# lifunudt/CORB-SLAM

Measured on AMD Instinct MI355X. Metric: stereo frames/sec ORB extract+match, higher is better.
Workload: dtype u8; 1 GPU; configs[1]: ORB extract+match, synthetic 1241x376 stereo stream, 2000 feat/frame, 8 levels x1.2, FAST 20/7; warmup_frames_per_gpu=2560, batches_in_flight=1, distinct_frames=64, parallelism=1 client per GPU, replicas (no collective), inputs=resident in HBM

## Files before the change

corb-slam_amd/csrc/corb_internal.h:

```cpp
#pragma once
#include <hip/hip_runtime.h>
#include <stdint.h>
#include <stddef.h>
#include "../../include/corb_accel.h"

#include <stdlib.h>
#ifdef CORB_DEV
static inline const char* corb_dev_env(const char* name) { return getenv(name); }
#else
static inline const char* corb_dev_env(const char*) { return nullptr; }
#endif

#define CORB_MAX_LEVELS 16
#define CORB_EDGE_THRESHOLD 19
#define CORB_MIN_BORDER 16
#define CORB_HALF_PATCH 15
#define CORB_PATCH_SIZE 31
#define CORB_TH_HIGH 100
#define CORB_TH_LOW 50
#define CORB_HISTO_LENGTH 30

struct CorbLevel {
    int w, h, pitch;
    int plane_off;
    int nCols, nRows, wCell, hCell;
    int maxBX, maxBY;
    int cell_base;
    int cell_cap;
    int cand_base;
    int cand_cap;
    int quota;
    int kp_base, kp_cap;
    int nIni;
    int node_cap;
    int blur_tile_base, blur_tiles_x, blur_tiles_y;
    int resize_tab_off;
    int resize_rec_off;
    float scale;
    float hX;
    int patch_size;
};

struct CorbFastCell {
    uint32_t src_off;
    uint32_t org;
    uint32_t dim;
    uint32_t lane;
};

#define CORB_BLUR_T 64
#define CORB_MAX_PARTS 4

struct CorbOrbParams {
    int nlevels, n_images;
    int img_base;
    int ini_th, min_th;
    int cells_per_image, cand_per_image, kp_per_image, out_cap;
    int blur_tiles_per_image;
    int node_cap_max, ncell_max;
    int fast_tp, fast_th;
    int pyr_strips;
    short pyr_r0[8][CORB_MAX_LEVELS], pyr_r1[8][CORB_MAX_LEVELS];
    int pyr_ctiles;
    short pyr_g0[8][CORB_MAX_LEVELS], pyr_g1[8][CORB_MAX_LEVELS];
    size_t arena_per_image;
    uint8_t* pyr;
    uint8_t* blur;
    int* cell_count;
    uint32_t* cand;
    uint32_t* keys;
    uint16_t* key_node;
    uint32_t* kp;
    int* kp_count;
    const short* resize_tab;
    const int2* resize_rec;
    const CorbFastCell* fast_cells;
    CorbKeyPoint* out_kp;
    uint8_t* out_desc;
    int* out_count;
    int* status;
    CorbLevel lv[CORB_MAX_LEVELS];
};

struct CorbStereoParams {
    int n_frames, nlevels;
    int frame_base;
    float bf, mb;
    float scale[CORB_MAX_LEVELS], inv_scale[CORB_MAX_LEVELS];
    int rows0;
    float* u_right;
    float* depth;
    int* sad;
    int* n_matched;
    int* row_off;
    int2* row_idx;
    int row_cap;
    int2* left_range;
};

#ifdef __HIPCC__
__device__ __forceinline__ void corb_xcd_remap(int& unit, int& img)
{
    const unsigned nx = gridDim.x, nimg = gridDim.y;
    const unsigned B = blockIdx.x + nx * blockIdx.y;
    const unsigned g = B / (8u * nx), r = B - g * 8u * nx;
    const unsigned in_group = min(8u, nimg - 8u * g);
    img = (int)(8u * g + r % in_group);
    unit = (int)(r / in_group);
}
#endif

struct CorbStereoDeviceFrame { const CorbKeyPoint* kp; const uint8_t* desc; const float* u_right; const float* depth; const int* count; int cap; hipStream_t stream; int device; };
struct CorbStereo;
int corb_stereo_device_frame(CorbStereo* h, int frame, CorbStereoDeviceFrame* out);
struct CorbRgbd;
int corb_rgbd_device_frame(CorbRgbd* h, int frame, CorbStereoDeviceFrame* out);

struct CorbProfiler;
void corb_orb_device_init();
void corb_launch_ingest(const uint8_t* stage, int w, int h, int n_images, uint8_t* plane, int pitch, size_t image_stride, hipStream_t stream);
void corb_launch_stereo_pack(const CorbOrbParams& p, const CorbStereoParams& s, int frame_base, int n_frames, uint8_t* out, const CorbStereoFrameLayout& lay, hipStream_t stream, struct CorbProfiler* prof);
void corb_launch_orb_pipeline(const CorbOrbParams& p, int img_base, int n_images, size_t octree_lds, hipStream_t stream, CorbProfiler* prof, hipEvent_t after_fast = nullptr);
void corb_launch_candidates(const CorbOrbParams* dp, int img, int level, CorbKeyPoint* out, int cap, int* n_out, hipStream_t stream);
void corb_launch_stereo(const CorbOrbParams& p, const CorbStereoParams& s, int frame_base, int n_frames, hipStream_t stream, CorbProfiler* prof);
size_t corb_octree_lds_bytes(int node_cap_max, int ncell_max);

#ifdef __HIPCC__
#include <hip/hip_ext.h>
#define CORB_LAUNCH(prof, name, kernel, grid, block, lds, stream, ...) do { \
// ... 19 lines not shown
```

corb-slam_amd/csrc/corb_orb.cpp:

```cpp
#include "corb_internal.h"
#include "orb_handle.h"
#include <cmath>
#include <cfloat>
#include <cstdio>
#include <cstdarg>
#include <cstring>
#include <mutex>
#include <map>
#include <vector>

static thread_local char g_err[512] = "";
void corb_set_error(const char* fmt, ...)
{
    va_list ap; va_start(ap, fmt); vsnprintf(g_err, sizeof(g_err), fmt, ap); va_end(ap);
}
extern "C" const char* corb_last_error(void) { return g_err; }
extern "C" int corb_version(void) { return 100; }
extern "C" int corb_abi_version(void) { return CORB_ABI_VERSION; }
extern "C" int corb_device_count(void)
{
    int n = 0;
    if (hipGetDeviceCount(&n) != hipSuccess) return 0;
    return n;
}
// ... 11 lines not shown

static inline int cv_round(double v) { return (int)lrint(v); }
static inline int cv_floor(double v) { int i = cv_round(v); float d = (float)(v - i); return i - (d < 0); }
static inline int cv_ceil(double v) { int i = cv_round(v); float d = (float)(i - v); return i + (d < 0); }
static inline short sat_short(int v) { return (short)(v < -32768 ? -32768 : v > 32767 ? 32767 : v); }

int corb_select_device(int device)
{
    int n = 0;
    if (hipGetDeviceCount(&n) != hipSuccess || n <= 0) { corb_set_error("no HIP device visible"); return CORB_ERR_NO_DEVICE; }
    if (device < 0 || device >= n) { corb_set_error("device %d out of range (%d visible)", device, n); return CORB_ERR_ARG; }
    HIPCHK(hipSetDevice(device));
    static std::mutex mu; static bool inited[64] = {false};
    std::lock_guard<std::mutex> lk(mu);
    if (device < 64 && !inited[device]) {
        hipDeviceProp_t prop;
        HIPCHK(hipGetDeviceProperties(&prop, device));
        if (strncmp(prop.gcnArchName, "gfx950", 6) != 0) {
            corb_set_error("device %d is %s; libcorb_accel is built for gfx950 only", device, prop.gcnArchName);
            return CORB_ERR_NO_DEVICE;
        }
        corb_orb_device_init();
        HIPCHK(hipGetLastError());
        inited[device] = true;
    }
    return CORB_OK;
}

static void build_resize_tables(int sw, int sh, int dw, int dh, short* tab)
{
    short* xofs = tab, * xa0 = tab + dw, * xa1 = tab + 2 * dw;
    short* ys0 = tab + 3 * dw, * ys1 = ys0 + dh, * yb0 = ys1 + dh, * yb1 = yb0 + dh;
    const double inv_scale_x = (double)dw / sw, inv_scale_y = (double)dh / sh;
    const double scale_x = 1. / inv_scale_x, scale_y = 1. / inv_scale_y;
    for (int dx = 0; dx < dw; dx++) {
        float fx = (float)((dx + 0.5) * scale_x - 0.5);
        int sx = cv_floor(fx);
        fx -= sx;
        if (sx < 0) { fx = 0; sx = 0; }
        if (sx + 1 >= sw) { if (sx >= sw - 1) { fx = 0; sx = sw - 1; } }
        xofs[dx] = (short)sx;
        xa0[dx] = sat_short(cv_round((1.f - fx) * 2048));
        xa1[dx] = sat_short(cv_round(fx * 2048));
        if (sx + 1 >= sw) { xa0[dx] = 2048; xa1[dx] = 0; }
    }
    for (int dy = 0; dy < dh; dy++) {
        float fy = (float)((dy + 0.5) * scale_y - 0.5);
        int sy = cv_floor(fy);
        fy -= sy;
        yb0[dy] = sat_short(cv_round((1.f - fy) * 2048));
        yb1[dy] = sat_short(cv_round(fy * 2048));
        ys0[dy] = (short)(sy < 0 ? 0 : (sy < sh ? sy : sh - 1));
        ys1[dy] = (short)(sy + 1 < 0 ? 0 : (sy + 1 < sh ? sy + 1 : sh - 1));
    }
}

extern "C" int corb_orb_create(const CorbOrbConfig* cfg, CorbOrb** out)
{
    if (!cfg || !out) { corb_set_error("null argument"); return CORB_ERR_ARG; }
    *out = nullptr;
    if (cfg->nlevels < 1 || cfg->nlevels > CORB_MAX_LEVELS || cfg->nfeatures < 1 || cfg->max_images < 1 ||
        cfg->width < 1 || cfg->height < 1 || cfg->width > 4000 || cfg->height > 4000 || !(cfg->scale_factor > 1.0f) ||
        cfg->min_th_fast < 1 || cfg->ini_th_fast < cfg->min_th_fast || cfg->ini_th_fast > 255) {
        corb_set_error("invalid CorbOrbConfig"); return CORB_ERR_ARG;
    }
    int rc = corb_select_device(cfg->device);
    if (rc != CORB_OK) return rc;
    CorbOrb* h = new CorbOrb();
    h->cfg = *cfg;
    const int nl = cfg->nlevels;
    h->scale[0] = 1.0f; h->sigma2[0] = 1.0f;
    for (int i = 1; i < nl; i++) { h->scale[i] = h->scale[i - 1] * cfg->scale_factor; h->sigma2[i] = h->scale[i] * h->scale[i]; }
    for (int i = 0; i < nl; i++) { h->inv_scale[i] = 1.0f / h->scale[i]; h->inv_sigma2[i] = 1.0f / h->sigma2[i]; }
    {
        float factor = 1.0f / cfg->scale_factor;
        float nDesired = cfg->nfeatures * (1 - factor) / (1 - (float)pow((double)factor, (double)nl));
        int sum = 0;
        for (int level = 0; level < nl - 1; level++) { h->quota[level] = cv_round(nDesired); sum += h->quota[level]; nDesired *= factor; }
        h->quota[nl - 1] = std::max(cfg->nfeatures - sum, 0);
        int v, v0, vmax = cv_floor(CORB_HALF_PATCH * sqrtf(2.f) / 2 + 1), vmin = cv_ceil(CORB_HALF_PATCH * sqrtf(2.f) / 2);
        const double hp2 = CORB_HALF_PATCH * CORB_HALF_PATCH;
        for (v = 0; v <= vmax; ++v) h->umax[v] = cv_round(sqrt(hp2 - v * v));
        for (v = CORB_HALF_PATCH, v0 = 0; v >= vmin; --v) { while (h->umax[v0] == h->umax[v0 + 1]) ++v0; h->umax[v] = v0; ++v0; }
        static const int expect[16] = {15, 15, 15, 15, 14, 14, 14, 13, 13, 12, 11, 10, 9, 8, 6, 3};
        for (int i = 0; i < 16; i++) if (h->umax[i] != expect[i]) { corb_set_error("umax table mismatch"); delete h; return CORB_ERR_ARG; }
    }
    CorbOrbParams& p = h->p;
    memset(&p, 0, sizeof(p));
    p.nlevels = nl; p.n_images = cfg->max_images; p.ini_th = cfg->ini_th_fast; p.min_th = cfg->min_th_fast;
    size_t arena = 0; int cells = 0, cands = 0, kps = 0, tiles = 0, tab_off = 0, rec_off = 0;
    for (int l = 0; l < nl; l++) {
        CorbLevel& L = p.lv[l];
        L.w = cv_round((float)cfg->width * h->inv_scale[l]);
        L.h = cv_round((float)cfg->height * h->inv_scale[l]);
        L.pitch = (L.w + 63) & ~63;
        L.plane_off = (int)arena;
        arena += ((size_t)L.pitch * L.h + 255) & ~(size_t)255;
        L.maxBX = L.w - CORB_EDGE_THRESHOLD + 3; L.maxBY = L.h - CORB_EDGE_THRESHOLD + 3;
        const float width = (float)(L.maxBX - CORB_MIN_BORDER), height = (float)(L.maxBY - CORB_MIN_BORDER);
        L.nCols = (int)(width / 30.f); L.nRows = (int)(height / 30.f);
        if (L.nCols < 1 || L.nRows < 1) { corb_set_error("level %d (%dx%d) too small for the 30-px FAST grid", l, L.w, L.h); delete h; return CORB_ERR_ARG; }
        L.wCell = (int)ceilf(width / L.nCols); L.hCell = (int)ceilf(height / L.nRows);
        if (L.wCell > 64 || L.hCell > 64) { corb_set_error("FAST cell %dx%d exceeds the LDS tile", L.wCell, L.hCell); delete h; return CORB_ERR_ARG; }
        L.cell_base = cells; cells += L.nCols * L.nRows;
        L.cell_cap = ((L.wCell + 1) / 2) * ((L.hCell + 1) / 2);
        L.cand_base = cands; L.cand_cap = L.nCols * L.nRows * L.cell_cap; cands += L.cand_cap;
// ... 20 lines not shown
    h->octree_lds = corb_octree_lds_bytes(p.node_cap_max, p.ncell_max);
    if (h->octree_lds > 160 * 1024) { corb_set_error("quadtree needs %zu B of LDS (> 160 KiB): nfeatures too large", h->octree_lds); delete h; return CORB_ERR_ARG; }
    if (p.node_cap_max > 65535) { corb_set_error("nfeatures too large"); delete h; return CORB_ERR_ARG; }
    const size_t NI = (size_t)cfg->max_images;
    short* d_tab = nullptr;
#define DA(ptr, n) do { rc = dalloc(h, &(ptr), (n)); if (rc != CORB_OK) { corb_orb_destroy(h); return rc; } } while (0)
    DA(p.pyr, NI * arena); DA(p.blur, NI * arena);
    DA(p.cell_count, NI * cells); DA(p.cand, NI * cands); DA(p.keys, NI * cands); DA(p.key_node, NI * cands);
    DA(p.kp, NI * kps); DA(p.kp_count, NI * CORB_MAX_LEVELS);
    DA(p.out_kp, NI * p.out_cap); DA(p.out_desc, NI * p.out_cap * 32); DA(p.out_count, NI); DA(p.status, NI);
    DA(d_tab, (size_t)tab_off);
    int2* d_rec = nullptr;
    DA(d_rec, (size_t)rec_off + 4);
    CorbFastCell* d_cells = nullptr;
    DA(d_cells, (size_t)cells);
    DA(h->dp, 1);
#undef DA
    p.resize_tab = d_tab;
    p.resize_rec = d_rec;
    p.fast_cells = d_cells;
    {
        std::vector<CorbFastCell> fc((size_t)cells);
        for (int l = 0; l < nl; l++) {
            const CorbLevel& L = p.lv[l];
            for (int c = 0; c < L.nCols * L.nRows; c++) {
                const int ci = c / L.nCols, cj = c - ci * L.nCols;
                const int iniX = CORB_MIN_BORDER + cj * L.wCell, iniY = CORB_MIN_BORDER + ci * L.hCell;
                const int cw = std::min(iniX + L.wCell + 6, L.maxBX) - iniX, ch = std::min(iniY + L.hCell + 6, L.maxBY) - iniY;
                CorbFastCell& f = fc[(size_t)L.cell_base + c];
                f.org = (uint32_t)(iniX + 3 - CORB_MIN_BORDER) | ((uint32_t)(iniY + 3 - CORB_MIN_BORDER) << 12) | ((uint32_t)l << 24);
                if (cw < 7 || ch < 7) { f.src_off = 0; f.org |= 0x80000000u; f.dim = 0; f.lane = 0; continue; }
                const int gx0 = iniX - 1, a = gx0 & 3, ng = (cw - 6 + 3) >> 2;
                f.src_off = (uint32_t)L.plane_off + (uint32_t)iniY * (uint32_t)L.pitch + (uint32_t)(gx0 - a);
                f.dim = (uint32_t)cw | ((uint32_t)ch << 8) | ((uint32_t)(64 / ng) << 16) | ((uint32_t)ng << 24);
                f.lane = (uint32_t)((65536 + ng - 1) / ng) | ((uint32_t)((a + cw) >> 2) << 20);
            }
        }
        if (hipMemcpy(d_cells, fc.data(), fc.size() * sizeof(CorbFastCell), hipMemcpyHostToDevice) != hipSuccess) { corb_set_error("FAST cell table upload failed"); corb_orb_destroy(h); return CORB_ERR_HIP; }
    }
    {
        std::vector<short> tab(tab_off);
        for (int l = 1; l < nl; l++) build_resize_tables(p.lv[l - 1].w, p.lv[l - 1].h, p.lv[l].w, p.lv[l].h, tab.data() + p.lv[l].resize_tab_off);
        std::vector<int2> rec((size_t)rec_off + 4, make_int2(0, 0));
        for (int l = 1; l < nl; l++) {
            const short* tl = tab.data() + p.lv[l].resize_tab_off; const int w = p.lv[l].w, hh = p.lv[l].h;
            int2* xr = rec.data() + p.lv[l].resize_rec_off; int2* yr = xr + ((w + 3) & ~3);
            for (int x = 0; x < ((w + 3) & ~3); x++) { const int xc = std::min(x, w - 1); xr[x] = make_int2(tl[xc], (int)(unsigned short)tl[w + xc] | ((int)(unsigned short)tl[2 * w + xc] << 16)); }
            const short* ys0 = tl + 3 * w; const short* ys1 = ys0 + hh; const short* yb0 = ys1 + hh; const short* yb1 = yb0 + hh;
            for (int y = 0; y < hh; y++) yr[y] = make_int2((int)(unsigned short)ys0[y] | ((int)(unsigned short)ys1[y] << 16), (int)(unsigned short)yb0[y] | ((int)(unsigned short)yb1[y] << 16));
        }
        if (hipMemcpy(d_rec, rec.data(), rec.size() * sizeof(int2), hipMemcpyHostToDevice) != hipSuccess) { corb_set_error("resize record upload failed"); corb_orb_destroy(h); return CORB_ERR_HIP; }
        const int S = 4;
        p.pyr_strips = (nl > 1 && p.lv[nl - 1].h >= 4 * S) ? S : 0;
        for (int s = 0; s < p.pyr_strips; s++) {
            int lo = 0, hi = 0;
            for (int l = nl - 1; l >= 1; l--) {
                const int blo = (int)((long long)s * p.lv[l].h / S), bhi = (int)((long long)(s + 1) * p.lv[l].h / S);
                if (l == nl - 1) { lo = blo; hi = bhi; }
                else {
                    const short* tl = tab.data() + p.lv[l + 1].resize_tab_off;
                    const short* ys0 = tl + 3 * p.lv[l + 1].w; const short* ys1 = ys0 + p.lv[l + 1].h;
                    const int clo = ys0[lo], chi = ys1[hi - 1] + 1;
                    lo = std::min(blo, clo); hi = std::max(bhi, chi);
                }
                p.pyr_r0[s][l] = (short)lo; p.pyr_r1[s][l] = (short)hi;
            }
        }
        const int C = 4;
        p.pyr_ctiles = (p.pyr_strips > 0 && p.lv[nl - 1].w >= 16 * C) ? C : 1;
        for (int c = 0; c < p.pyr_ctiles; c++) {
            int lo = 0, hi = 0;
            for (int l = nl - 1; l >= 1; l--) {
                const int ng = (p.lv[l].w + 3) / 4;
                const int blo = (int)((long long)c * ng / p.pyr_ctiles), bhi = (int)((long long)(c + 1) * ng / p.pyr_ctiles);
                if (l == nl - 1) { lo = blo; hi = bhi; }
                else {
                    const short* xofs = tab.data() + p.lv[l + 1].resize_tab_off;
                    const int wn = p.lv[l + 1].w, x_first = std::min(4 * lo, wn - 1), x_last = std::min(4 * hi, wn) - 1;
                    const int clo = xofs[x_first] / 4, chi = std::min(xofs[x_last] + 1, p.lv[l].w - 1) / 4 + 1;
                    lo = std::min(blo, clo); hi = std::max(bhi, chi);
                }
                p.pyr_g0[c][l] = (short)lo; p.pyr_g1[c][l] = (short)hi;
            }
        }
        if (hipMemcpy(d_tab, tab.data(), tab.size() * sizeof(short), hipMemcpyHostToDevice) != hipSuccess ||
            hipMemcpy(h->dp, &p, sizeof(p), hipMemcpyHostToDevice) != hipSuccess ||
            hipMemset(p.status, 0, NI * sizeof(int)) != hipSuccess || hipMemset(p.out_count, 0, NI * sizeof(int)) != hipSuccess ||
            hipMemset(p.pyr, 0, NI * arena) != hipSuccess || hipMemset(p.blur, 0, NI * arena) != hipSuccess ||
            hipStreamCreateWithFlags(&h->stream, hipStreamNonBlocking) != hipSuccess ||
            hipHostMalloc((void**)&h->h_status, NI * sizeof(int)) != hipSuccess ||
            hipHostMalloc((void**)&h->h_count, NI * sizeof(int)) != hipSuccess ||
            hipMalloc((void**)&h->d_stage, (size_t)cfg->width * cfg->height + 256) != hipSuccess ||
            hipHostMalloc((void**)&h->h_img, (size_t)cfg->width * cfg->height) != hipSuccess ||
            hipHostMalloc((void**)&h->h_kp, (size_t)p.out_cap * sizeof(CorbKeyPoint)) != hipSuccess ||
            hipHostMalloc((void**)&h->h_desc, (size_t)p.out_cap * 32) != hipSuccess ||
            hipHostMalloc((void**)&h->h_f32, (size_t)p.out_cap * 2 * sizeof(float)) != hipSuccess ||
            hipHostMalloc((void**)&h->h_misc, 8 * sizeof(int)) != hipSuccess) {
            corb_set_error("device initialisation failed: %s", hipGetErrorString(hipGetLastError()));
            corb_orb_destroy(h); return CORB_ERR_HIP;
        }
    }
    if (const char* e = getenv("CORB_PARTS")) h->parts = std::max(1, std::min(CORB_MAX_PARTS, atoi(e)));
    for (int i = 0; i < CORB_MAX_PARTS; i++)
        if (hipEventCreateWithFlags(&h->ev_stage[i], hipEventDisableTiming) != hipSuccess) { corb_set_error("event creation failed: %s", hipGetErrorString(hipGetLastError())); corb_orb_destroy(h); return CORB_ERR_HIP; }
    *out = h;
    return CORB_OK;
}

extern "C" void corb_orb_destroy(CorbOrb* h)
{
    if (!h) return;
    (void)hipSetDevice(h->cfg.device);
    if (h->stream) { (void)hipStreamSynchronize(h->stream); (void)hipStreamDestroy(h->stream); }
    for (int i = 0; i < CORB_MAX_PARTS - 1; i++) {
        if (h->side[i]) { (void)hipStreamSynchronize(h->side[i]); (void)hipStreamDestroy(h->side[i]); }
        if (h->ev_done[i]) (void)hipEventDestroy(h->ev_done[i]);
    }
    for (int i = 0; i < CORB_MAX_PARTS; i++) if (h->ev_stage[i]) (void)hipEventDestroy(h->ev_stage[i]);
    for (void* ptr : h->allocs) (void)hipFree(ptr);
    if (h->h_status) (void)hipHostFree(h->h_status);
    if (h->h_count) (void)hipHostFree(h->h_count);
    if (h->d_stage) (void)hipFree(h->d_stage);
    if (h->d_stage_batch) (void)hipFree(h->d_stage_batch);
    if (h->h_img) (void)hipHostFree(h->h_img);
    if (h->h_kp) (void)hipHostFree(h->h_kp);
    if (h->h_desc) (void)hipHostFree(h->h_desc);
    if (h->h_f32) (void)hipHostFree(h->h_f32);
    if (h->h_misc) (void)hipHostFree(h->h_misc);
    if (h->d_cand_tmp) (void)hipFree(h->d_cand_tmp);
    if (h->d_cand_n) (void)hipFree(h->d_cand_n);
    delete h;
}

extern "C" int corb_orb_tables(const CorbOrb* h, float* scale, float* inv_scale, float* sigma2, float* inv_sigma2,
                               int32_t* features_per_level, int32_t* umax)
{
    if (!h) return CORB_ERR_ARG;
// ... 433 lines not shown
```

corb-slam_amd/csrc/orb_kernels.hip:

```cpp
#include "corb_internal.h"
#include "lane_exchange.h"
#include <atomic>
#include <cstring>
#include <cstdlib>
#include "brief_pattern.h"

#define WAVE 64

struct CorbDescribeTab { uint4 patb[64]; };
__device__ CorbDescribeTab g_dsc_tab;


#define RS_ROWS 8
__global__ __launch_bounds__(256) void orb_resize_kernel(const CorbOrbParams p, int level)
{
    const CorbLevel& D = p.lv[level];
    const CorbLevel& S = p.lv[level - 1];
    const int img = p.img_base + blockIdx.z;
    const int x4 = (blockIdx.x * 64 + threadIdx.x) * 4;
    const int yb = (blockIdx.y * 4 + threadIdx.y) * RS_ROWS;
    if (x4 >= D.w || yb >= D.h) return;
    const short* tab = p.resize_tab + D.resize_tab_off;
    const short* xofs = tab, * xa0 = tab + D.w, * xa1 = tab + 2 * D.w;
    const short* ys0 = tab + 3 * D.w, * ys1 = ys0 + D.h, * yb0 = ys1 + D.h, * yb1 = yb0 + D.h;
// ... 18 lines not shown
        for (int k = 0; k < 4; k++) {
            const int d0 = __mul24(S0[sx[k]], a0[k]) + __mul24(S0[sx1[k]], a1[k]);
            const int d1 = __mul24(S1[sx[k]], a0[k]) + __mul24(S1[sx1[k]], a1[k]);
            const uint32_t v = (uint32_t)((((__mul24(b0, d0 >> 4)) >> 16) + ((__mul24(b1, d1 >> 4)) >> 16) + 2) >> 2) & 0xFFu;
            packed |= v << (8 * k);
        }
        uint8_t* dst = dstp + (size_t)y * D.pitch + x4;
        if (nvalid == 4) *reinterpret_cast<uint32_t*>(dst) = packed;
        else for (int k = 0; k < nvalid; k++) dst[k] = (uint8_t)(packed >> (8 * k));
    }
}

__device__ __forceinline__ uint32_t mul24u(uint32_t a, uint32_t b) { uint32_t d; asm("v_mul_u32_u24 %0, %1, %2" : "=v"(d) : "v"(a), "v"(b)); return d; }
__device__ __forceinline__ uint32_t mad24u(uint32_t a, uint32_t b, uint32_t c) { uint32_t d; asm("v_mad_u32_u24 %0, %1, %2, %3" : "=v"(d) : "v"(a), "v"(b), "v"(c)); return d; }
template <int B> __device__ __forceinline__ uint32_t mul24_byte(uint32_t packed, uint32_t b)
{
    uint32_t d;
    if constexpr (B == 0) asm("v_mul_u32_u24_sdwa %0, %1, %2 dst_sel:DWORD dst_unused:UNUSED_PAD src0_sel:BYTE_0 src1_sel:DWORD" : "=v"(d) : "v"(packed), "v"(b));
    if constexpr (B == 1) asm("v_mul_u32_u24_sdwa %0, %1, %2 dst_sel:DWORD dst_unused:UNUSED_PAD src0_sel:BYTE_1 src1_sel:DWORD" : "=v"(d) : "v"(packed), "v"(b));
    if constexpr (B == 2) asm("v_mul_u32_u24_sdwa %0, %1, %2 dst_sel:DWORD dst_unused:UNUSED_PAD src0_sel:BYTE_2 src1_sel:DWORD" : "=v"(d) : "v"(packed), "v"(b));
    if constexpr (B == 3) asm("v_mul_u32_u24_sdwa %0, %1, %2 dst_sel:DWORD dst_unused:UNUSED_PAD src0_sel:BYTE_3 src1_sel:DWORD" : "=v"(d) : "v"(packed), "v"(b));
    return d;
}
__device__ __forceinline__ uint32_t mul24_hiword(uint32_t a, uint32_t b)
{ uint32_t d; asm("v_mul_u32_u24_sdwa %0, %1, %2 dst_sel:DWORD dst_unused:UNUSED_PAD src0_sel:WORD_1 src1_sel:DWORD" : "=v"(d) : "v"(a), "v"(b)); return d; }
__device__ __forceinline__ uint32_t add_hiwords(uint32_t a, uint32_t b)
{ uint32_t d; asm("v_add_u32_sdwa %0, %1, %2 dst_sel:DWORD dst_unused:UNUSED_PAD src0_sel:WORD_1 src1_sel:WORD_1" : "=v"(d) : "v"(a), "v"(b)); return d; }
template <int B> __device__ __forceinline__ void shr_into_byte(uint32_t& packed, uint32_t sh, uint32_t x)
{
    if constexpr (B == 0) asm("v_lshrrev_b32_sdwa %0, %1, %2 dst_sel:BYTE_0 dst_unused:UNUSED_PRESERVE src0_sel:DWORD src1_sel:DWORD" : "+v"(packed) : "v"(sh), "v"(x));
    if constexpr (B == 1) asm("v_lshrrev_b32_sdwa %0, %1, %2 dst_sel:BYTE_1 dst_unused:UNUSED_PRESERVE src0_sel:DWORD src1_sel:DWORD" : "+v"(packed) : "v"(sh), "v"(x));
    if constexpr (B == 2) asm("v_lshrrev_b32_sdwa %0, %1, %2 dst_sel:BYTE_2 dst_unused:UNUSED_PRESERVE src0_sel:DWORD src1_sel:DWORD" : "+v"(packed) : "v"(sh), "v"(x));
    if constexpr (B == 3) asm("v_lshrrev_b32_sdwa %0, %1, %2 dst_sel:BYTE_3 dst_unused:UNUSED_PRESERVE src0_sel:DWORD src1_sel:DWORD" : "+v"(packed) : "v"(sh), "v"(x));
}
__device__ __forceinline__ int pick_byte(uint32_t w0, uint32_t w1, uint32_t w2, int o)
{
    const uint32_t a = o < 4 ? w0 : (o < 8 ? w1 : w2);
    return (int)((a >> ((o & 3) * 8)) & 255u);
}

template <int K> __device__ __forceinline__ void pyr_px(uint32_t& packed, uint32_t P0, uint32_t P1, uint32_t Q0, uint32_t Q1,
                                                         uint32_t A0, uint32_t A1, uint32_t b0, uint32_t b1, uint32_t two)
{
    const uint32_t d0 = mul24_byte<K>(P0, A0) + mul24_byte<K>(P1, A1);
    const uint32_t d1 = mul24_byte<K>(Q0, A0) + mul24_byte<K>(Q1, A1);
    const uint32_t m0 = mul24_hiword(d0, b0), m1 = mul24_hiword(d1, b1);
    shr_into_byte<K>(packed, two, add_hiwords(m0, m1) + 2u);
}

#define PYR_T 256
typedef const uint64_t __attribute__((address_space(4)))* pyr_yrec_ptr;
struct PyrUni { static constexpr bool value = true; };
struct PyrLane { static constexpr bool value = false; };
__device__ __forceinline__ int pyr_chunk_width(int rem)
{
    if (rem >= 64) return 64;
    return (64 / rem) * rem * 4 >= 3 * 64 ? rem : 1 << (31 - __clz(rem));
}
__global__ __launch_bounds__(PYR_T, 8) void orb_pyramid_kernel(const CorbOrbParams p)
{
    const int strip = blockIdx.x / p.pyr_ctiles, ctile = blockIdx.x - strip * p.pyr_ctiles, img = p.img_base + blockIdx.y;
    uint8_t* base = p.pyr + (size_t)img * p.arena_per_image;
    const uint32_t two = 2u;
    const int wave = __builtin_amdgcn_readfirstlane((int)threadIdx.x >> 6), lane = (int)threadIdx.x & 63;
    for (int level = 1; level < p.nlevels; level++) {
        const CorbLevel& D = p.lv[level];
        const CorbLevel& S = p.lv[level - 1];
        const int2* xrec = p.resize_rec + D.resize_rec_off;
        const pyr_yrec_ptr yrec = (pyr_yrec_ptr)(uintptr_t)(xrec + ((D.w + 3) & ~3));
        const uint8_t* src = base + S.plane_off;
        uint8_t* dstp = base + D.plane_off;
        const int r0 = p.pyr_r0[strip][level], r1 = p.pyr_r1[strip][level];
        const int gfirst = p.pyr_g0[ctile][level], gend = p.pyr_g1[ctile][level];
        const int wq = (r1 - r0 + 3) >> 2, wr0 = r0 + wave * wq, wr1 = min(wr0 + wq, r1);
        for (int gbase = gfirst, W = 0; gbase < gend && wr0 < wr1; gbase += W) {
            W = pyr_chunk_width(gend - gbase);
            const int R = 64 / W, len = (wr1 - wr0 + R - 1) / R;
            const int run = lane / W, tx = lane - run * W;
            const int y0 = wr0 + run * len, y1 = min(y0 + len, wr1);
            if (run >= R || y0 >= y1) continue;
            const int x4 = (gbase + tx) * 4;
            int sx[4], sx1[4];
            uint32_t A0[4], A1[4];
            int nvalid = 0;
            const int4 xr01 = *reinterpret_cast<const int4*>(xrec + x4), xr23 = *reinterpret_cast<const int4*>(xrec + x4 + 2);
            const int xs[4] = {xr01.x, xr01.z, xr23.x, xr23.z}, xa[4] = {xr01.y, xr01.w, xr23.y, xr23.w};
#pragma unroll
            for (int k = 0; k < 4; k++) {
                sx[k] = xs[k]; sx1[k] = min(sx[k] + 1, S.w - 1);
                A0[k] = (uint32_t)(xa[k] & 0xFFFF) << 12; A1[k] = (uint32_t)(xa[k] >> 16) << 12;
                nvalid += (x4 + k < D.w) ? 1 : 0;
            }
            const int bx = sx[0] & ~3;
            const bool wide = (sx1[3] - bx) < 12;
            uint32_t s1a = 0, s2a = 0, s1b = 0, s2b = 0;
#pragma unroll
            for (int k = 0; k < 4; k++) {
                const int oa = sx[k] - bx, ob = sx1[k] - bx;
                s1a |= (uint32_t)(oa < 8 ? oa : 0x0c) << (8 * k); s2a |= (uint32_t)(oa < 8 ? k : oa - 4) << (8 * k);
                s1b |= (uint32_t)(ob < 8 ? ob : 0x0c) << (8 * k); s2b |= (uint32_t)(ob < 8 ? k : ob - 4) << (8 * k);
            }
            if (wide) {
                auto hpass = [&](const uint32_t (&w)[3], uint32_t (&d)[4]) {
                    const uint32_t P0 = __builtin_amdgcn_perm(w[2], __builtin_amdgcn_perm(w[1], w[0], s1a), s2a), P1 = __builtin_amdgcn_perm(w[2], __builtin_amdgcn_perm(w[1], w[0], s1b), s2b);
                    d[0] = mul24_byte<0>(P0, A0[0]) + mul24_byte<0>(P1, A1[0]); d[1] = mul24_byte<1>(P0, A0[1]) + mul24_byte<1>(P1, A1[1]);
                    d[2] = mul24_byte<2>(P0, A0[2]) + mul24_byte<2>(P1, A1[2]); d[3] = mul24_byte<3>(P0, A0[3]) + mul24_byte<3>(P1, A1[3]);
                };
                auto rows = [&](auto mode) {
                    constexpr bool UNI = decltype(mode)::value;
                    auto uni = [](int v) { if constexpr (UNI) return __builtin_amdgcn_readfirstlane(v); else return v; };
                    auto rec = [&](int yy) { const uint64_t v = yrec[yy]; return make_uint2((uint32_t)v, (uint32_t)(v >> 32)); };
                    auto fresh = [](uint32_t s0, uint32_t kept) -> bool { if constexpr (UNI) return s0 != kept; else return __any(s0 != kept) != 0; };
                    auto load_row = [&](uint32_t s, uint32_t (&w)[3]) {
                        const uint32_t* q;
                        if constexpr (UNI) q = reinterpret_cast<const uint32_t*>(src + s * (uint32_t)S.pitch + (uint32_t)bx);
                        else q = reinterpret_cast<const uint32_t*>(src + (uint32_t)(__mul24((int)s, S.pitch) + bx));
                        w[0] = q[0]; w[1] = q[1]; w[2] = q[2];
                    };
                    uint32_t dk[4] = {0u, 0u, 0u, 0u};
                    uint32_t kept = 0xFFFFu;
                    auto emit = [&](int yy, bool fr, const uint32_t (&t)[3], const uint32_t (&b)[3], uint32_t bb) {
                        const uint32_t b0 = bb & 0xFFFFu, b1 = bb >> 16;
                        uint32_t dt[4];
                        if (fr) hpass(t, dt);
                        else { dt[0] = dk[0]; dt[1] = dk[1]; dt[2] = dk[2]; dt[3] = dk[3]; }
                        hpass(b, dk);
                        uint32_t packed = 0;
                        shr_into_byte<0>(packed, two, add_hiwords(mul24_hiword(dt[0], b0), mul24_hiword(dk[0], b1)) + 2u);
                        shr_into_byte<1>(packed, two, add_hiwords(mul24_hiword(dt[1], b0), mul24_hiword(dk[1], b1)) + 2u);
                        shr_into_byte<2>(packed, two, add_hiwords(mul24_hiword(dt[2], b0), mul24_hiword(dk[2], b1)) + 2u);
                        shr_into_byte<3>(packed, two, add_hiwords(mul24_hiword(dt[3], b0), mul24_hiword(dk[3], b1)) + 2u);
                        uint8_t* dst;
                        if constexpr (UNI) dst = dstp + (uint32_t)yy * (uint32_t)D.pitch + (uint32_t)x4;
                        else dst = dstp + (uint32_t)(__mul24(yy, D.pitch) + x4);
                        if (nvalid == 4) *reinterpret_cast<uint32_t*>(dst) = packed;
                        else for (int k = 0; k < nvalid; k++) dst[k] = (uint8_t)(packed >> (8 * k));
                    };
                    int y = uni(y0);
                    const int yend = uni(y1), ylast = r1 - 1;
                    uint2 ra = rec(min(y, ylast)), rb = rec(min(y + 1, ylast));
                    if constexpr (UNI) {
                        uint2 rc = rec(min(y + 2, ylast)), rd = rec(min(y + 3, ylast));
#pragma unroll 1
                        for (; y + 3 < yend; y += 4) {
                            uint32_t ta[3], tb[3], tc[3], td[3], ba[3], bb[3], bc[3], bd[3];
                            const bool fa = fresh(ra.x & 0xFFFFu, kept), fb = fresh(rb.x & 0xFFFFu, ra.x >> 16), fc = fresh(rc.x & 0xFFFFu, rb.x >> 16), fd = fresh(rd.x & 0xFFFFu, rc.x >> 16);
                            if (fa) load_row(ra.x & 0xFFFFu, ta);
                            load_row(ra.x >> 16, ba);
                            if (fb) load_row(rb.x & 0xFFFFu, tb);
                            load_row(rb.x >> 16, bb);
                            if (fc) load_row(rc.x & 0xFFFFu, tc);
                            load_row(rc.x >> 16, bc);
                            if (fd) load_row(rd.x & 0xFFFFu, td);
                            load_row(rd.x >> 16, bd);
                            const uint2 na = rec(min(y + 4, ylast)), nb = rec(min(y + 5, ylast)), nc = rec(min(y + 6, ylast)), nd = rec(min(y + 7, ylast));
                            emit(y, fa, ta, ba, ra.y); emit(y + 1, fb, tb, bb, rb.y); emit(y + 2, fc, tc, bc, rc.y); emit(y + 3, fd, td, bd, rd.y);
                            kept = rd.x >> 16;
                            ra = na; rb = nb; rc = nc; rd = nd;
                        }
                    }
#pragma unroll 1
                    for (; y + 1 < yend; y += 2) {
                        uint32_t ta[3], tb[3], ba[3], bb[3];
                        const bool fa = fresh(ra.x & 0xFFFFu, kept), fb = fresh(rb.x & 0xFFFFu, ra.x >> 16);
                        if (fa) load_row(ra.x & 0xFFFFu, ta);
                        load_row(ra.x >> 16, ba);
                        if (fb) load_row(rb.x & 0xFFFFu, tb);
                        load_row(rb.x >> 16, bb);
                        const uint2 na = rec(min(y + 2, ylast)), nb = rec(min(y + 3, ylast));
                        emit(y, fa, ta, ba, ra.y); emit(y + 1, fb, tb, bb, rb.y);
                        kept = rb.x >> 16;
                        ra = na; rb = nb;
                    }
                    if (y < yend) {
                        uint32_t ta[3], ba[3];
                        const bool fa = fresh(ra.x & 0xFFFFu, kept);
                        if (fa) load_row(ra.x & 0xFFFFu, ta);
                        load_row(ra.x >> 16, ba);
                        emit(y, fa, ta, ba, ra.y);
                    }
                };
                if (R == 1) rows(PyrUni{}); else rows(PyrLane{});
            } else {
#pragma unroll 1
                for (int y = y0; y < y1; y++) {
                    const uint64_t yv = yrec[y];
                    const int2 yr = make_int2((int)(uint32_t)yv, (int)(uint32_t)(yv >> 32));
                    const uint8_t* S0 = src + (uint32_t)__mul24(yr.x & 0xFFFF, S.pitch);
                    const uint8_t* S1 = src + (uint32_t)__mul24(yr.x >> 16, S.pitch);
                    const uint32_t b0 = yr.y & 0xFFFF, b1 = (uint32_t)yr.y >> 16;
                    uint32_t packed = 0;
#pragma unroll
                    for (int k = 0; k < 4; k++) {
                        const uint32_t d0 = mad24u(S0[sx[k]], A0[k] >> 12, mul24u(S0[sx1[k]], A1[k] >> 12));
                        const uint32_t d1 = mad24u(S1[sx[k]], A0[k] >> 12, mul24u(S1[sx1[k]], A1[k] >> 12));
                        const uint32_t v = (((mul24u(b0, d0 >> 4) >> 16) + (mul24u(b1, d1 >> 4) >> 16) + 2u) >> 2) & 0xFFu;
                        packed |= v << (8 * k);
                    }
                    uint8_t* dst = dstp + (uint32_t)(__mul24(y, D.pitch) + x4);
                    if (nvalid == 4) *reinterpret_cast<uint32_t*>(dst) = packed;
                    else for (int k = 0; k < nvalid; k++) dst[k] = (uint8_t)(packed >> (8 * k));
                }
            }
        }
        __threadfence_block();
        __syncthreads();
    }
}


__device__ __forceinline__ uint32_t pk_min3(uint32_t a, uint32_t b, uint32_t c)
{ uint32_t d; asm("v_pk_minimum3_f16 %0, %1, %2, %3" : "=v"(d) : "v"(a), "v"(b), "v"(c)); return d; }
__device__ __forceinline__ uint32_t pk_max3(uint32_t a, uint32_t b, uint32_t c)
{ uint32_t d; asm("v_pk_maximum3_f16 %0, %1, %2, %3" : "=v"(d) : "v"(a), "v"(b), "v"(c)); return d; }
template <int K> __device__ __forceinline__ uint32_t pk_pair(const uint32_t (&w)[3])
{
    static_assert(K >= 0 && K <= 10, "window");
    if constexpr (K <= 6) return __builtin_amdgcn_perm(w[1], w[0], 0x0c000c00u | (uint32_t)K | ((uint32_t)(K + 1) << 16));
    else return __builtin_amdgcn_perm(w[2], w[1], 0x0c000c00u | (uint32_t)(K - 4) | ((uint32_t)(K - 3) << 16));
}
typedef short corb_short2 __attribute__((ext_vector_type(2)));

template <bool BRIGHT> __device__ __forceinline__ uint32_t fast_arc_chain(const uint32_t (&v)[16])
{
    auto in3 = [](uint32_t a, uint32_t b, uint32_t c) { return BRIGHT ? pk_min3(a, b, c) : pk_max3(a, b, c); };
    auto out3 = [](uint32_t a, uint32_t b, uint32_t c) { return BRIGHT ? pk_max3(a, b, c) : pk_min3(a, b, c); };
    uint32_t w3[16], w9[16], r5[5];
#pragma unroll
    for (int i = 0; i < 16; i++) w3[i] = in3(v[i], v[(i + 1) & 15], v[(i + 2) & 15]);
#pragma unroll
    for (int i = 0; i < 16; i++) w9[i] = in3(w3[i], w3[(i + 3) & 15], w3[(i + 6) & 15]);
#pragma unroll
    for (int i = 0; i < 5; i++) r5[i] = out3(w9[3 * i], w9[3 * i + 1], w9[3 * i + 2]);
    return out3(out3(r5[0], r5[1], r5[2]), out3(r5[3], r5[4], w9[15]), r5[0]);
}

template <int J> __device__ __forceinline__ uint32_t fast_pair_score(const uint32_t (&R)[7][3], uint32_t th2, uint32_t kb, uint32_t kd)
{
    constexpr int C = 4 + 2 * J;
    uint32_t v[16];
    v[0] = pk_pair<C>(R[6]);      v[1] = pk_pair<C + 1>(R[6]);  v[2] = pk_pair<C + 2>(R[5]);  v[3] = pk_pair<C + 3>(R[4]);
    v[4] = pk_pair<C + 3>(R[3]);  v[5] = pk_pair<C + 3>(R[2]);  v[6] = pk_pair<C + 2>(R[1]);  v[7] = pk_pair<C + 1>(R[0]);
    v[8] = pk_pair<C>(R[0]);      v[9] = pk_pair<C - 1>(R[0]);  v[10] = pk_pair<C - 2>(R[1]); v[11] = pk_pair<C - 3>(R[2]);
    v[12] = pk_pair<C - 3>(R[3]); v[13] = pk_pair<C - 3>(R[4]); v[14] = pk_pair<C - 2>(R[5]); v[15] = pk_pair<C - 1>(R[6]);
    const uint32_t cpk = pk_pair<C>(R[3]);
    const uint32_t e0 = pk_max3(v[0], v[8], v[8]), e1 = pk_max3(v[4], v[12], v[12]), f0 = pk_min3(v[0], v[8], v[8]), f1 = pk_min3(v[4], v[12], v[12]);
    const uint32_t m = pk_min3(e0, e1, e1), n = pk_max3(f0, f1, f1);
    const uint32_t nbright = (cpk + kb) - m;
    const uint32_t dark = ((cpk + kd) - n) & 0x02000200u;
    const uint32_t donly = dark & nbright, both = dark ^ donly;
    const uint32_t xm = (donly >> 1) - (donly >> 9);
#pragma unroll
    for (int i = 0; i < 16; i++) v[i] ^= xm;
    const corb_short2 c = __builtin_bit_cast(corb_short2, cpk ^ xm) + (short)1;
// ... 1014 lines not shown
```

Before: 109,600 stereo frames/s.

## Precompute pyramid resize chunk and column tables on host

Moves the per-wave chunk partitioning and the per-column resize setup (source offsets, byte-permute selectors, weights, wide flag) out of the pyramid kernel into host-built tables stored in device memory. The kernel then walks a list of chunk descriptors through scalar loads and reads each column descriptor as four 16-byte vector loads, instead of recomputing them in every block. The partial-store loop is also unrolled into explicit byte stores. The aim is to cut scalar and vector ALU setup work in the pyramid kernel, paid for with extra memory reads of the descriptor tables and more init-time setup.

```diff
diff --git a/corb-slam_amd/csrc/corb_internal.h b/corb-slam_amd/csrc/corb_internal.h
--- a/corb-slam_amd/csrc/corb_internal.h
+++ b/corb-slam_amd/csrc/corb_internal.h
@@ -48,6 +48,19 @@
     uint32_t lane;
 };
 
+struct CorbPyrChunk {
+    uint32_t col0;
+    uint32_t shape;
+    uint32_t rows;
+    uint32_t len;
+};
+struct CorbPyrCol {
+    uint32_t bx, nvalid;
+    uint32_t s1a, s2a, s1b, s2b;
+    uint32_t x4, pad;
+    uint32_t A0[4], A1[4];
+};
+
 #define CORB_BLUR_T 64
 #define CORB_MAX_PARTS 4
 
@@ -60,9 +73,7 @@
     int node_cap_max, ncell_max;
     int fast_tp, fast_th;
     int pyr_strips;
-    short pyr_r0[8][CORB_MAX_LEVELS], pyr_r1[8][CORB_MAX_LEVELS];
     int pyr_ctiles;
-    short pyr_g0[8][CORB_MAX_LEVELS], pyr_g1[8][CORB_MAX_LEVELS];
     size_t arena_per_image;
     uint8_t* pyr;
     uint8_t* blur;
@@ -75,6 +86,9 @@
     const short* resize_tab;
     const int2* resize_rec;
     const CorbFastCell* fast_cells;
+    const uint2* pyr_work;
+    const CorbPyrChunk* pyr_chunks;
+    const CorbPyrCol* pyr_cols;
     CorbKeyPoint* out_kp;
     uint8_t* out_desc;
     int* out_count;
diff --git a/corb-slam_amd/csrc/corb_orb.cpp b/corb-slam_amd/csrc/corb_orb.cpp
--- a/corb-slam_amd/csrc/corb_orb.cpp
+++ b/corb-slam_amd/csrc/corb_orb.cpp
@@ -87,6 +87,56 @@
         yb1[dy] = sat_short(cv_round(fy * 2048));
         ys0[dy] = (short)(sy < 0 ? 0 : (sy < sh ? sy : sh - 1));
         ys1[dy] = (short)(sy + 1 < 0 ? 0 : (sy + 1 < sh ? sy + 1 : sh - 1));
+    }
+}
+
+static int pyr_chunk_width(int rem)
+{
+    if (rem >= 64) return 64;
+    if ((64 / rem) * rem * 4 >= 3 * 64) return rem;
+    int w = 1;
+    while (2 * w <= rem) w *= 2;
+    return w;
+}
+
+static void build_pyr_cols(int sw, int w, const short* xofs, const short* xa0, const short* xa1, CorbPyrCol* cols, std::vector<char>& wide)
+{
+    const int ng = (w + 3) / 4;
+    wide.assign((size_t)ng, 0);
+    for (int g = 0; g < ng; g++) {
+        CorbPyrCol& c = cols[g];
+        memset(&c, 0, sizeof(c));
+        int sx[4], sx1[4];
+        for (int k = 0; k < 4; k++) {
+            const int x = std::min(4 * g + k, w - 1);
+            sx[k] = xofs[x]; sx1[k] = std::min(sx[k] + 1, sw - 1);
+            c.A0[k] = (uint32_t)(unsigned short)xa0[x] << 12; c.A1[k] = (uint32_t)(unsigned short)xa1[x] << 12;
+            c.nvalid += (4 * g + k < w) ? 1 : 0;
+        }
+        const int bx = sx[0] & ~3;
+        c.bx = (uint32_t)bx; c.x4 = (uint32_t)(4 * g);
+        wide[(size_t)g] = (sx1[3] - bx) < 12;
+        for (int k = 0; k < 4; k++) {
+            const int oa = sx[k] - bx, ob = sx1[k] - bx;
+            c.s1a |= (uint32_t)(oa < 8 ? oa : 0x0c) << (8 * k); c.s2a |= (uint32_t)(oa < 8 ? k : (oa - 4) & 7) << (8 * k);
+            c.s1b |= (uint32_t)(ob < 8 ? ob : 0x0c) << (8 * k); c.s2b |= (uint32_t)(ob < 8 ? k : (ob - 4) & 7) << (8 * k);
+        }
+    }
+}
+
+static void build_pyr_chunks(int g0, int g1, int wr0, int wr1, int r1, int col_off, const std::vector<char>& wide, std::vector<CorbPyrChunk>& chunks)
+{
+    for (int gbase = g0, W = 0; gbase < g1 && wr0 < wr1; gbase += W) {
+        W = pyr_chunk_width(g1 - gbase);
+        const int R = 64 / W, len = (wr1 - wr0 + R - 1) / R;
+        bool all_wide = true;
+        for (int g = gbase; g < gbase + W; g++) all_wide = all_wide && wide[(size_t)g];
+        CorbPyrChunk c;
+        c.col0 = (uint32_t)(col_off + gbase);
+        c.shape = (uint32_t)((65536 + W - 1) / W) | ((uint32_t)W << 17) | ((uint32_t)R << 24) | ((uint32_t)all_wide << 31);
+        c.rows = (uint32_t)wr0 | ((uint32_t)wr1 << 16);
+        c.len = (uint32_t)len | ((uint32_t)(r1 - 1) << 16);
+        chunks.push_back(c);
     }
 }
 
@@ -213,6 +263,8 @@
         if (hipMemcpy(d_rec, rec.data(), rec.size() * sizeof(int2), hipMemcpyHostToDevice) != hipSuccess) { corb_set_error("resize record upload failed"); corb_orb_destroy(h); return CORB_ERR_HIP; }
         const int S = 4;
         p.pyr_strips = (nl > 1 && p.lv[nl - 1].h >= 4 * S) ? S : 0;
+        short pyr_r0[4][CORB_MAX_LEVELS], pyr_r1[4][CORB_MAX_LEVELS];
+        short pyr_g0[4][CORB_MAX_LEVELS], pyr_g1[4][CORB_MAX_LEVELS];
         for (int s = 0; s < p.pyr_strips; s++) {
             int lo = 0, hi = 0;
             for (int l = nl - 1; l >= 1; l--) {
@@ -224,7 +276,7 @@
                     const int clo = ys0[lo], chi = ys1[hi - 1] + 1;
                     lo = std::min(blo, clo); hi = std::max(bhi, chi);
                 }
-                p.pyr_r0[s][l] = (short)lo; p.pyr_r1[s][l] = (short)hi;
+                pyr_r0[s][l] = (short)lo; pyr_r1[s][l] = (short)hi;
             }
         }
         const int C = 4;
@@ -241,9 +293,39 @@
                     const int clo = xofs[x_first] / 4, chi = std::min(xofs[x_last] + 1, p.lv[l].w - 1) / 4 + 1;
                     lo = std::min(blo, clo); hi = std::max(bhi, chi);
                 }
-                p.pyr_g0[c][l] = (short)lo; p.pyr_g1[c][l] = (short)hi;
+                pyr_g0[c][l] = (short)lo; pyr_g1[c][l] = (short)hi;
             }
         }
+        std::vector<CorbPyrCol> cols; std::vector<CorbPyrChunk> chunks;
+        std::vector<uint2> work((size_t)std::max(p.pyr_strips * p.pyr_ctiles, 1) * CORB_MAX_LEVELS * 4, make_uint2(0u, 0u));
+        if (p.pyr_strips > 0) {
+            int col_off[CORB_MAX_LEVELS] = {0};
+            std::vector<std::vector<char>> wide((size_t)nl);
+            for (int l = 1; l < nl; l++) {
+                const short* tl = tab.data() + p.lv[l].resize_tab_off; const int w = p.lv[l].w;
+                col_off[l] = (int)cols.size(); cols.resize(cols.size() + (size_t)(w + 3) / 4);
+                build_pyr_cols(p.lv[l - 1].w, w, tl, tl + w, tl + 2 * w, cols.data() + col_off[l], wide[(size_t)l]);
+            }
+            for (int s = 0; s < p.pyr_strips; s++)
+                for (int c = 0; c < p.pyr_ctiles; c++)
+                    for (int l = 1; l < nl; l++) {
+                        const int r0 = pyr_r0[s][l], r1 = pyr_r1[s][l], wq = (r1 - r0 + 3) >> 2;
+                        for (int wave = 0; wave < 4; wave++) {
+                            const int wr0 = r0 + wave * wq, wr1 = std::min(wr0 + wq, r1);
+                            const size_t first = chunks.size();
+                            build_pyr_chunks(pyr_g0[c][l], pyr_g1[c][l], wr0, wr1, r1, col_off[l], wide[(size_t)l], chunks);
+                            work[((size_t)(s * p.pyr_ctiles + c) * CORB_MAX_LEVELS + l) * 4 + wave] = make_uint2((uint32_t)first, (uint32_t)(chunks.size() - first));
+                        }
+                    }
+        }
+        if (cols.empty()) cols.resize(1);
+        if (chunks.empty()) chunks.resize(1);
+        uint2* d_work = nullptr; CorbPyrChunk* d_chunks = nullptr; CorbPyrCol* d_cols = nullptr;
+        if (dalloc(h, &d_work, work.size()) || dalloc(h, &d_chunks, chunks.size()) || dalloc(h, &d_cols, cols.size())) { corb_orb_destroy(h); return CORB_ERR_HIP; }
+        p.pyr_work = d_work; p.pyr_chunks = d_chunks; p.pyr_cols = d_cols;
+        if (hipMemcpy(d_work, work.data(), work.size() * sizeof(uint2), hipMemcpyHostToDevice) != hipSuccess ||
+            hipMemcpy(d_chunks, chunks.data(), chunks.size() * sizeof(CorbPyrChunk), hipMemcpyHostToDevice) != hipSuccess ||
+            hipMemcpy(d_cols, cols.data(), cols.size() * sizeof(CorbPyrCol), hipMemcpyHostToDevice) != hipSuccess) { corb_set_error("pyramid work table upload failed"); corb_orb_destroy(h); return CORB_ERR_HIP; }
         if (hipMemcpy(d_tab, tab.data(), tab.size() * sizeof(short), hipMemcpyHostToDevice) != hipSuccess ||
             hipMemcpy(h->dp, &p, sizeof(p), hipMemcpyHostToDevice) != hipSuccess ||
             hipMemset(p.status, 0, NI * sizeof(int)) != hipSuccess || hipMemset(p.out_count, 0, NI * sizeof(int)) != hipSuccess ||
diff --git a/corb-slam_amd/csrc/orb_kernels.hip b/corb-slam_amd/csrc/orb_kernels.hip
--- a/corb-slam_amd/csrc/orb_kernels.hip
+++ b/corb-slam_amd/csrc/orb_kernels.hip
@@ -94,14 +94,13 @@
 typedef const uint64_t __attribute__((address_space(4)))* pyr_yrec_ptr;
 struct PyrUni { static constexpr bool value = true; };
 struct PyrLane { static constexpr bool value = false; };
-__device__ __forceinline__ int pyr_chunk_width(int rem)
-{
-    if (rem >= 64) return 64;
-    return (64 / rem) * rem * 4 >= 3 * 64 ? rem : 1 << (31 - __clz(rem));
-}
+typedef uint32_t pyr_u32x2 __attribute__((ext_vector_type(2)));
+typedef uint32_t pyr_u32x4 __attribute__((ext_vector_type(4)));
+typedef const pyr_u32x2 __attribute__((address_space(4)))* pyr_work_ptr;
+typedef const pyr_u32x4 __attribute__((address_space(4)))* pyr_chunk_ptr;
 __global__ __launch_bounds__(PYR_T, 8) void orb_pyramid_kernel(const CorbOrbParams p)
 {
-    const int strip = blockIdx.x / p.pyr_ctiles, ctile = blockIdx.x - strip * p.pyr_ctiles, img = p.img_base + blockIdx.y;
+    const int img = p.img_base + blockIdx.y;
     uint8_t* base = p.pyr + (size_t)img * p.arena_per_image;
     const uint32_t two = 2u;
     const int wave = __builtin_amdgcn_readfirstlane((int)threadIdx.x >> 6), lane = (int)threadIdx.x & 63;
@@ -112,36 +111,20 @@
         const pyr_yrec_ptr yrec = (pyr_yrec_ptr)(uintptr_t)(xrec + ((D.w + 3) & ~3));
         const uint8_t* src = base + S.plane_off;
         uint8_t* dstp = base + D.plane_off;
-        const int r0 = p.pyr_r0[strip][level], r1 = p.pyr_r1[strip][level];
-        const int gfirst = p.pyr_g0[ctile][level], gend = p.pyr_g1[ctile][level];
-        const int wq = (r1 - r0 + 3) >> 2, wr0 = r0 + wave * wq, wr1 = min(wr0 + wq, r1);
-        for (int gbase = gfirst, W = 0; gbase < gend && wr0 < wr1; gbase += W) {
-            W = pyr_chunk_width(gend - gbase);
-            const int R = 64 / W, len = (wr1 - wr0 + R - 1) / R;
-            const int run = lane / W, tx = lane - run * W;
+        const pyr_u32x2 work = ((pyr_work_ptr)(uintptr_t)p.pyr_work)[((int)blockIdx.x * CORB_MAX_LEVELS + level) * (PYR_T / WAVE) + wave];
+        for (uint32_t c = work.x, cend = work.x + work.y; c < cend; c++) {
+            const pyr_u32x4 ck = ((pyr_chunk_ptr)(uintptr_t)p.pyr_chunks)[c];
+            const int W = (int)((ck.y >> 17) & 127u), R = (int)((ck.y >> 24) & 127u);
+            const bool wide = (ck.y >> 31) != 0u;
+            const int wr0 = (int)(ck.z & 0xFFFFu), wr1 = (int)(ck.z >> 16), len = (int)(ck.w & 0xFFFFu), ylast = (int)(ck.w >> 16);
+            const int run = (int)(((uint32_t)lane * (ck.y & 0x1FFFFu)) >> 16), tx = lane - run * W;
             const int y0 = wr0 + run * len, y1 = min(y0 + len, wr1);
             if (run >= R || y0 >= y1) continue;
-            const int x4 = (gbase + tx) * 4;
-            int sx[4], sx1[4];
-            uint32_t A0[4], A1[4];
-            int nvalid = 0;
-            const int4 xr01 = *reinterpret_cast<const int4*>(xrec + x4), xr23 = *reinterpret_cast<const int4*>(xrec + x4 + 2);
-            const int xs[4] = {xr01.x, xr01.z, xr23.x, xr23.z}, xa[4] = {xr01.y, xr01.w, xr23.y, xr23.w};
-#pragma unroll
-            for (int k = 0; k < 4; k++) {
-                sx[k] = xs[k]; sx1[k] = min(sx[k] + 1, S.w - 1);
-                A0[k] = (uint32_t)(xa[k] & 0xFFFF) << 12; A1[k] = (uint32_t)(xa[k] >> 16) << 12;
-                nvalid += (x4 + k < D.w) ? 1 : 0;
-            }
-            const int bx = sx[0] & ~3;
-            const bool wide = (sx1[3] - bx) < 12;
-            uint32_t s1a = 0, s2a = 0, s1b = 0, s2b = 0;
-#pragma unroll
-            for (int k = 0; k < 4; k++) {
-                const int oa = sx[k] - bx, ob = sx1[k] - bx;
-                s1a |= (uint32_t)(oa < 8 ? oa : 0x0c) << (8 * k); s2a |= (uint32_t)(oa < 8 ? k : oa - 4) << (8 * k);
-                s1b |= (uint32_t)(ob < 8 ? ob : 0x0c) << (8 * k); s2b |= (uint32_t)(ob < 8 ? k : ob - 4) << (8 * k);
-            }
+            const uint4* colp = reinterpret_cast<const uint4*>(p.pyr_cols + ck.x + (uint32_t)tx);
+            const uint4 c0 = colp[0], c1 = colp[1], c2 = colp[2], c3 = colp[3];
+            const int bx = (int)c0.x, nvalid = (int)c0.y, x4 = (int)c1.z;
+            const uint32_t s1a = c0.z, s2a = c0.w, s1b = c1.x, s2b = c1.y;
+            const uint32_t A0[4] = {c2.x, c2.y, c2.z, c2.w}, A1[4] = {c3.x, c3.y, c3.z, c3.w};
             if (wide) {
                 auto hpass = [&](const uint32_t (&w)[3], uint32_t (&d)[4]) {
                     const uint32_t P0 = __builtin_amdgcn_perm(w[2], __builtin_amdgcn_perm(w[1], w[0], s1a), s2a), P1 = __builtin_amdgcn_perm(w[2], __builtin_amdgcn_perm(w[1], w[0], s1b), s2b);
@@ -150,7 +133,6 @@
                 };
                 auto rows = [&](auto mode) {
                     constexpr bool UNI = decltype(mode)::value;
-                    auto uni = [](int v) { if constexpr (UNI) return __builtin_amdgcn_readfirstlane(v); else return v; };
                     auto rec = [&](int yy) { const uint64_t v = yrec[yy]; return make_uint2((uint32_t)v, (uint32_t)(v >> 32)); };
                     auto fresh = [](uint32_t s0, uint32_t kept) -> bool { if constexpr (UNI) return s0 != kept; else return __any(s0 != kept) != 0; };
                     auto load_row = [&](uint32_t s, uint32_t (&w)[3]) {
@@ -176,10 +158,14 @@
                         if constexpr (UNI) dst = dstp + (uint32_t)yy * (uint32_t)D.pitch + (uint32_t)x4;
                         else dst = dstp + (uint32_t)(__mul24(yy, D.pitch) + x4);
                         if (nvalid == 4) *reinterpret_cast<uint32_t*>(dst) = packed;
-                        else for (int k = 0; k < nvalid; k++) dst[k] = (uint8_t)(packed >> (8 * k));
+                        else {
+                            dst[0] = (uint8_t)packed;
+                            if (nvalid > 1) dst[1] = (uint8_t)(packed >> 8);
+                            if (nvalid > 2) dst[2] = (uint8_t)(packed >> 16);
+                        }
                     };
-                    int y = uni(y0);
-                    const int yend = uni(y1), ylast = r1 - 1;
+                    int y = UNI ? wr0 : y0;
+                    const int yend = UNI ? wr1 : y1;
                     uint2 ra = rec(min(y, ylast)), rb = rec(min(y + 1, ylast));
                     if constexpr (UNI) {
                         uint2 rc = rec(min(y + 2, ylast)), rd = rec(min(y + 3, ylast));
@@ -224,6 +210,9 @@
                 };
                 if (R == 1) rows(PyrUni{}); else rows(PyrLane{});
             } else {
+                const int4 xr01 = *reinterpret_cast<const int4*>(xrec + x4), xr23 = *reinterpret_cast<const int4*>(xrec + x4 + 2);
+                const int sx[4] = {xr01.x, xr01.z, xr23.x, xr23.z};
+                const int sx1[4] = {min(sx[0] + 1, S.w - 1), min(sx[1] + 1, S.w - 1), min(sx[2] + 1, S.w - 1), min(sx[3] + 1, S.w - 1)};
 #pragma unroll 1
                 for (int y = y0; y < y1; y++) {
                     const uint64_t yv = yrec[y];
@@ -241,7 +230,11 @@
                     }
                     uint8_t* dst = dstp + (uint32_t)(__mul24(y, D.pitch) + x4);
                     if (nvalid == 4) *reinterpret_cast<uint32_t*>(dst) = packed;
-                    else for (int k = 0; k < nvalid; k++) dst[k] = (uint8_t)(packed >> (8 * k));
+                    else {
+                        dst[0] = (uint8_t)packed;
+                        if (nvalid > 1) dst[1] = (uint8_t)(packed >> 8);
+                        if (nvalid > 2) dst[2] = (uint8_t)(packed >> 16);
+                    }
                 }
             }
         }
```

Result: faster. 110,900 stereo frames/s (median of 6 runs) (+1.2%).
